# roymor1/OptimalStrategiesAgainstGenerativeAttacks

Measured on AMD Instinct MI355X. Metric: GIM episodes/sec (64x64x3, m=1 n=5 k=10), higher is better.
Workload: dtype f32

## Files before the change

### include/gim_hip.h

```cpp
#ifndef GIM_HIP_H
#define GIM_HIP_H

#include <stddef.h>
#include <stdint.h>

#ifdef __cplusplus
extern "C" {
#endif

#define GIM_OK 0
#define GIM_E_BADARG (-1)
#define GIM_E_LAUNCH (-2)

const char* gim_last_error(void);
int gim_version(void);

typedef struct {
    int32_t N, H, W, Cin, Cout, KH, ups;
    float pre_slope;
    int32_t pool, wfold, res_ups;
    int32_t tune_tile, tune_ksplit, tune_wgrad;
    int32_t out_zeroed;
    float post_slope;
    int32_t prec;
} gim_conv_shape;

int gim_conv2d_fold_weights(const float* w, float* f, int Cout, int Cin, int KH, void* stream);
typedef struct {
    const float* w;
    float* f;
    int32_t Cout, Cin, KH, reserved;
} gim_fold_job;
int gim_conv2d_fold_weights_batched(const gim_fold_job* jobs, const int32_t* tab, int n_blocks, void* stream);

int gim_conv2d_fwd(const float* x, const float* w, const float* bias, const float* sigma, const float* residual,
                   float* y, const gim_conv_shape* s, void* stream);

int gim_conv2d_dgrad(const float* dy, const float* w, const float* sigma, const float* mask_x, float* dx,
                     const gim_conv_shape* s, void* stream);

int gim_conv2d_dgrad_res(const float* dy, const float* w, const float* sigma, const float* mask_x, const float* res_half,
                         float res_scale, float* dx, const gim_conv_shape* s, void* stream);

int gim_conv2d_wgrad_slabs(const gim_conv_shape* s);
int gim_conv2d_wgrad(const float* dy, const float* x, float* slabs, float* bias_slabs, int n_slabs, const gim_conv_shape* s,
                     void* stream);

int gim_wgrad_finish(const float* slabs, const float* bias_slabs, int n_slabs, const float* w, const float* sigma,
                     const float* u, const float* v, float* dw, float* db, float* scratch, int Cout, int Cin, int KH,
                     int fold, float* acc_dw, float* acc_db, void* stream);

int gim_spectral_sigma(const float* w, float* u, float* v, float* sigma, float* u_out, float* v_out, float* scratch,
                       int Cout, int Cin, int KH, int training, void* stream);

typedef struct {
    const float* w;
    float* u;
    float* v;
    int64_t off_sigma, off_u, off_v, off_scratch;
    int32_t Cout, Cin, KH, reserved;
} gim_sn_job;
int gim_spectral_sigma_batched(const gim_sn_job* jobs, int n_jobs, const int32_t* tab_cols, int n_col_blocks,
                               const int32_t* tab_rows, int n_row_blocks, float* out_base, int training, void* stream);

int gim_conv2d_transpose_weights(const float* w, float* wt, int Cout, int Cin, int KF, void* stream);
int gim_conv2d_dgrad_t(const float* dy, const float* wt, const float* sigma, const float* mask_x, float* dx,
                       const gim_conv_shape* shape, void* stream);

int gim_conv2d_xfold_weights(const float* w, float* wx, int Cout, int Cin, int KH, int J, void* stream);
int gim_conv2d_dgrad_xfold(const float* dy, const float* wx, const float* sigma, const float* mask_x, float* dx,
                           const gim_conv_shape* shape, int J, void* stream);

int gim_pad_image(const float* x, float* xp, int N, int H, int W, int C, int pad, float slope, void* stream);
int gim_conv2d_pack_rows_weights(const float* w, float* wp, int Cout, int Cin, int KH, void* stream);
int gim_conv2d_fwd_rows(const float* xp, const float* wp, const float* bias, const float* sigma, const float* residual,
                        float* y, const gim_conv_shape* shape, void* stream);
int gim_conv2d_wgrad_rows_acc(const float* dy, const float* xp, float* acc, float* bias_acc, const gim_conv_shape* shape, void* stream);

int gim_conv2d_pack_subpixel_weights(const float* wf, float* wm, int Cout, int Cin, int KH, void* stream);
int gim_depth_to_space2(const float* y4, const float* bias, float* y, int N, int Hs, int Ws, int C, float post_slope, void* stream);

int gim_conv_launch_plan(const gim_conv_shape* shape, int kind, int32_t* out);

int gim_conv2d_wgrad_acc(const float* dy, const float* x, float* acc, float* bias_acc, const gim_conv_shape* shape, void* stream);

typedef struct {
    const float* src;
    const float* bias_src;
    const float* w;
    const float* sigma;
    const float* u;
    const float* v;
    float* tmp;
    float* partial;
    float* grad_w;
    float* grad_b;
    int32_t Cout, Cin, K, fold;
    int32_t n_chunks, exclusive;
} gim_wgrad_job;
int gim_wgrad_finish_batched(const gim_wgrad_job* jobs, int n_jobs, const int32_t* tab, int n_blocks, const int32_t* tab_sn,
                             int n_blocks_sn, void* stream);

int gim_colsum(const float* x, float* out, float* scratch, int64_t rows, int C, void* stream);

int gim_colsum_acc(const float* x, float* out, float* scratch, int64_t rows, int C, void* stream);
int gim_colsum2(const float* a, const float* b, float* out_a, float* out_b, int rows, int C, int accumulate, void* stream);

int gim_norm_fwd(const float* x, const float* scale, const float* shift, const float* residual, float* y, float* stats,
                 int N, int HW, int C, int mode, float eps, void* stream);
int gim_norm_fwd_act(const float* x, const float* scale, const float* shift, const float* residual, float* y, float* stats,
                     int N, int HW, int C, int mode, float eps, float post_slope, void* stream);
int gim_norm_bwd(const float* dy, const float* x, const float* scale, const float* stats, float* dx, float* dscale_nc,
                 float* dshift_nc, int N, int HW, int C, int mode, void* stream);

int gim_avgpool2_fwd(const float* x, float* y, int N, int H, int W, int C, void* stream);
int gim_avgpool2_fwd_act(const float* x, float* y, int N, int H, int W, int C, float in_slope, void* stream);
int gim_add_n(const float* a, const float* b, const float* c, const float* d, float* out, int64_t n, void* stream);
int gim_add_avgpool2_bwd(const float* g, const float* dy_pooled, float* out, int N, int H, int W, int C, void* stream);
int gim_avgpool2_bwd(const float* dy, float* dx, int N, int H, int W, int C, void* stream);
int gim_upsample2x_bwd(const float* dy_up, const float* mask_x, float slope, float* dx, int N, int H, int W, int C, void* stream);

int gim_maxpool_lrelu_fwd(const float* x, float* y, int32_t* idx, int N, int HW, int C, float slope, void* stream);
int gim_maxpool_lrelu_bwd(const float* dy, const float* y, const int32_t* idx, float* dx, int N, int HW, int C, float slope, void* stream);

int gim_attn_prob_fwd(const float* f, const float* g, float* P, int batch, int T, int K, void* stream);

int gim_bgemm(const float* A, const float* B, float* C, int batch, int M, int N, int K,
              int64_t sAb, int64_t sAi, int64_t sAk, int64_t sBb, int64_t sBk, int64_t sBj, void* stream);

typedef struct {
    const float* A;
    const float* B;
    float* C;
    const float* bias;
    int32_t M, N, K, ldc;
    int64_t sAi, sAk, sBk, sBj;
    int32_t flags, reserved;
} gim_gemm_job;
int gim_bgemm_grouped(const gim_gemm_job* jobs, const int32_t* tiles, int n_tiles, void* stream);
int gim_colsum_grouped(const gim_gemm_job* jobs, const int32_t* tiles, int n_tiles, void* stream);

int gim_softmax_dim1_fwd(const float* s, float* p, int B, int R, int Ccols, void* stream);
int gim_softmax_dim1_bwd(const float* dp, const float* p, float* ds, int B, int R, int Ccols, void* stream);

// ... 89 lines not shown
```

### optimalstrategiesagainstgenerativeattacks_amd/_lib.py

```python
import ctypes
import os
from ctypes import POINTER, c_float, c_int, c_int32, c_int64, c_void_p

_HERE = os.path.dirname(os.path.abspath(__file__))
LIB_PATH = os.environ.get("GIM_LIB_PATH") or os.path.join(_HERE, "csrc", "libgim_hip.so")


class GimConvShape(ctypes.Structure):
    _fields_ = [("N", c_int32), ("H", c_int32), ("W", c_int32), ("Cin", c_int32), ("Cout", c_int32),
                ("KH", c_int32), ("ups", c_int32), ("pre_slope", c_float),
                ("pool", c_int32), ("wfold", c_int32), ("res_ups", c_int32),
                ("tune_tile", c_int32), ("tune_ksplit", c_int32), ("tune_wgrad", c_int32),
                ("out_zeroed", c_int32), ("post_slope", c_float), ("prec", c_int32)]


class GimInferConv(ctypes.Structure):
    _fields_ = [("N", c_int32), ("H", c_int32), ("W", c_int32), ("Cin", c_int32), ("Cout", c_int32),
                ("KH", c_int32), ("stride", c_int32)]


P = c_void_p
SP = POINTER(GimConvShape)


class GimFoldJob(ctypes.Structure):
    _fields_ = [("w", P), ("f", P), ("Cout", c_int32), ("Cin", c_int32), ("KH", c_int32), ("reserved", c_int32)]


class GimSnJob(ctypes.Structure):
    _fields_ = [("w", P), ("u", P), ("v", P), ("off_sigma", c_int64), ("off_u", c_int64), ("off_v", c_int64), ("off_scratch", c_int64),
                ("Cout", c_int32), ("Cin", c_int32), ("KH", c_int32), ("reserved", c_int32)]


class GimWgradJob(ctypes.Structure):
    _fields_ = [("src", P), ("bias_src", P), ("w", P), ("sigma", P), ("u", P), ("v", P), ("tmp", P), ("partial", P),
                ("grad_w", P), ("grad_b", P), ("Cout", c_int32), ("Cin", c_int32), ("K", c_int32), ("fold", c_int32),
                ("n_chunks", c_int32), ("exclusive", c_int32)]


class GimGemmJob(ctypes.Structure):
    _fields_ = [("A", P), ("B", P), ("C", P), ("bias", P), ("M", c_int32), ("N", c_int32), ("K", c_int32), ("ldc", c_int32),
                ("sAi", c_int64), ("sAk", c_int64), ("sBk", c_int64), ("sBj", c_int64), ("flags", c_int32), ("reserved", c_int32)]


SIGNATURES = {
    "gim_conv2d_fwd": [P, P, P, P, P, P, SP, P],
    "gim_conv2d_dgrad": [P, P, P, P, P, SP, P],
    "gim_conv2d_dgrad_res": [P, P, P, P, P, c_float, P, SP, P],
    "gim_conv2d_wgrad_slabs": [SP],
    "gim_conv2d_wgrad": [P, P, P, P, c_int, SP, P],
    "gim_wgrad_finish": [P, P, c_int, P, P, P, P, P, P, P, c_int, c_int, c_int, c_int, P, P, P],
    "gim_conv2d_fold_weights": [P, P, c_int, c_int, c_int, P],
    "gim_conv2d_fold_weights_batched": [P, P, c_int, P],
    "gim_spectral_sigma": [P, P, P, P, P, P, P, c_int, c_int, c_int, c_int, P],
    "gim_spectral_sigma_batched": [P, c_int, P, c_int, P, c_int, P, c_int, P],
    "gim_colsum": [P, P, P, c_int64, c_int, P],
    "gim_norm_fwd": [P, P, P, P, P, P, c_int, c_int, c_int, c_int, c_float, P],
    "gim_norm_fwd_act": [P, P, P, P, P, P, c_int, c_int, c_int, c_int, c_float, c_float, P],
    "gim_norm_bwd": [P, P, P, P, P, P, P, c_int, c_int, c_int, c_int, P],
    "gim_avgpool2_fwd": [P, P, c_int, c_int, c_int, c_int, P],
    "gim_avgpool2_fwd_act": [P, P, c_int, c_int, c_int, c_int, c_float, P],
    "gim_add_n": [P, P, P, P, P, c_int64, P],
    "gim_add_avgpool2_bwd": [P, P, P, c_int, c_int, c_int, c_int, P],
    "gim_avgpool2_bwd": [P, P, c_int, c_int, c_int, c_int, P],
    "gim_upsample2x_bwd": [P, P, c_float, P, c_int, c_int, c_int, c_int, P],
    "gim_maxpool_lrelu_fwd": [P, P, P, c_int, c_int, c_int, c_float, P],
    "gim_maxpool_lrelu_bwd": [P, P, P, P, c_int, c_int, c_int, c_float, P],
    "gim_bgemm": [P, P, P, c_int, c_int, c_int, c_int, c_int64, c_int64, c_int64, c_int64, c_int64, c_int64, P],
    "gim_attn_prob_fwd": [P, P, P, c_int, c_int, c_int, P],
    "gim_softmax_dim1_fwd": [P, P, c_int, c_int, c_int, P],
    "gim_softmax_dim1_bwd": [P, P, P, c_int, c_int, c_int, P],
    "gim_bgemm_grouped": [P, P, c_int, P],
    "gim_colsum_grouped": [P, P, c_int, P],
    "gim_scale_add_fwd": [P, P, P, P, c_int64, P],
    "gim_scale_add_fwd_act": [P, P, P, P, c_int64, c_float, P],
    "gim_scale_add_bwd": [P, P, P, P, P, P, c_int64, P],
    "gim_tanh_fwd": [P, P, c_int64, P],
    "gim_tanh_bwd": [P, P, P, c_int64, P],
    "gim_nchw_to_nhwc": [P, P, c_int, c_int, c_int, P],
    "gim_nhwc_to_nchw": [P, P, c_int, c_int, c_int, P],
    "gim_set_stats_fwd": [P, P, P, c_int, c_int, c_int, c_int64, c_int64, P],
    "gim_set_stats_bwd": [P, P, P, P, c_int, c_int, c_int, c_int64, c_int64, P],
    "gim_bce_logits_fwd": [P, P, c_float, c_int, P],
    "gim_bce_logits_bwd": [P, P, P, c_float, c_int, P],
    "gim_sum_dim1": [P, P, c_int, c_int, c_int, c_float, P],
    "gim_repeat_dim1": [P, P, c_int, c_int, c_int, c_float, P],
    "gim_noise_combine": [P, P, P, c_int, c_int, c_int, c_int, P],
    "gim_concat2": [P, P, P, c_int64, c_int, c_int, c_int, c_int, P],
    "gim_slice_channels": [P, P, c_int64, c_int, c_int, P],
    "gim_conv2d_wgrad_acc": [P, P, P, P, SP, P],
    "gim_wgrad_finish_batched": [P, c_int, P, c_int, P, c_int, P],
    "gim_colsum_acc": [P, P, P, c_int64, c_int, P],
    "gim_colsum2": [P, P, P, P, c_int, c_int, c_int, P],
    "gim_conv_launch_plan": [SP, c_int, P],
    "gim_conv2d_transpose_weights": [P, P, c_int, c_int, c_int, P],
    "gim_conv2d_dgrad_t": [P, P, P, P, P, SP, P],
    "gim_conv2d_xfold_weights": [P, P, c_int, c_int, c_int, c_int, P],
    "gim_conv2d_dgrad_xfold": [P, P, P, P, P, SP, c_int, P],
    "gim_episode_gather": [P, P, P, P, c_int, c_int, c_int, c_int, P],
    "gim_resize_bilinear_u8": [P, c_int64, c_int, c_int, c_int, c_int, P, c_int, c_int, P, P, c_int, P, P, c_int, P],
    "gim_maxpool_gather": [P, P, P, P, c_int, c_int, c_int, c_float, P],
    "gim_softmax_dim1_bwd_dp": [P, P, P, P, c_int, c_int, c_int, P],
    "gim_set_stats_bwd_bwd": [P, P, P, P, P, P, c_int, c_int, c_int, c_int64, c_int64, P],
    "gim_lrelu_mask_mul": [P, P, c_float, P, c_int64, P],
    "gim_sqsum_rows_fwd": [P, P, c_int, c_int64, P],
    "gim_sqsum_rows_bwd": [P, P, P, c_int, c_int64, P],
    "gim_img_att_mix_fwd": [P, P, P, P, P, P, P, P, c_int64, c_int, P],
    "gim_img_att_mix_bwd": [P, P, P, P, P, P, P, P, P, P, P, P, P, P, c_int64, c_int, P],
    "gim_adam_step": [P, P, P, P, c_int64, P, P, c_int, c_float, c_float, c_float, c_float, P, P],
    "gim_adam_step_scaled": [P, P, P, P, c_int64, P, P, c_int, c_float, c_float, c_float, c_float, P, P, P],
    "gim_spin": [c_int, P],
    "gim_pad_image": [P, P, c_int, c_int, c_int, c_int, c_int, c_float, P],
    "gim_conv2d_pack_rows_weights": [P, P, c_int, c_int, c_int, P],
    "gim_conv2d_pack_subpixel_weights": [P, P, c_int, c_int, c_int, P],
    "gim_depth_to_space2": [P, P, P, c_int, c_int, c_int, c_int, c_float, P],
    "gim_conv2d_fwd_rows": [P, P, P, P, P, P, SP, P],
    "gim_conv2d_wgrad_rows_acc": [P, P, P, P, SP, P],
    "gim_conv2d_infer": [P, P, P, P, P, POINTER(GimInferConv), P],
    "gim_maxpool2_act": [P, P, c_int, c_int, c_int, c_int, c_int, P],
    "gim_channel_affine": [P, P, P, P, c_int64, c_int, P],
    "gim_se_tail": [P, P, P, P, P, P, P, c_int, c_int, c_int, c_int, c_int, P],
    "gim_pair_score": [P, P, P, c_int, c_int, P],
    "gim_l2norm_rows": [P, P, c_int, c_int, P],
    "gim_absdiff": [P, P, P, c_int64, P],
    "gim_bn_slabs": [c_int64],
    "gim_bn_partials_floats": [c_int64, c_int],
    "gim_bn_stats": [P, P, P, P, P, P, P, c_int64, c_int, c_float, c_float, P],
    "gim_bn_relu_maxpool2_fwd": [P, P, P, P, P, P, c_int, c_int, c_int, c_int, P],
    "gim_bn_pool_bwd_reduce": [P, P, P, P, P, P, P, P, P, P, P, c_int, c_int, c_int, c_int, P],
    "gim_bn_pool_bwd_dx": [P, P, P, P, P, P, P, P, P, c_int, c_int, c_int, c_int, P],
    "gim_absdiff_bwd": [P, P, P, P, P, c_int64, P],
    "gim_logit_accuracy": [P, c_int, c_int, P, P],
    "gim_version": [],
}

_lib = None


# ... 24 lines not shown
```

### optimalstrategiesagainstgenerativeattacks_amd/csrc/spectral.hip

```cpp
#include "common.h"

#define SN_R 8

__global__ __launch_bounds__(256) void sn_colpart_kernel(const float* __restrict__ w, const float* __restrict__ u,
                                                         float* __restrict__ part, int Cout, int K, int rows_per) {
    const int p = blockIdx.x * 256 + threadIdx.x;
    const int r = blockIdx.y;
    const int c0 = r * rows_per, c1 = min(Cout, c0 + rows_per);
    if (p >= K) return;
    float acc = 0.f;
    for (int co = c0; co < c1; ++co) acc += w[(long long)co * K + p] * u[co];
    part[(long long)r * K + p] = acc;
}

__global__ __launch_bounds__(256) void sn_vnorm_kernel(const float* __restrict__ part, int R, float* __restrict__ v,
                                                       float* __restrict__ v_phys, float* __restrict__ v_out, int K, int Cin,
                                                       int T, int training) {
    __shared__ float red[4];
    if (training) {
        float ss = 0.f;
        for (int p = threadIdx.x; p < K; p += 256) {
            float a = 0.f;
            for (int r = 0; r < R; ++r) a += part[(long long)r * K + p];
            v_phys[p] = a;
// ... 137 lines not shown
        const int kh = (int)(rr % K);
        const int co = (int)(rr / K);
        float g = 0.f;
#pragma unroll
        for (int dh = 0; dh < 2; ++dh)
#pragma unroll
            for (int dwd = 0; dwd < 2; ++dwd) {
                const int a = kh + dh, b = kw + dwd;
                if (fold == 1) g += src[(((long long)co * KF + a) * KF + b) * Cin + ci];
                else g += src[(((long long)ci * KF + (K - a)) * KF + (K - b)) * Cout + co];
            }
        if (fold == 1) g *= 0.25f;
        dw[i] = g;
        if (w) dot += g * w[i];
    }
    if (partial) {
        dot = block_sum_256(dot, red);
        if (threadIdx.x == 0) partial[blockIdx.x] = dot;
    }
}

__global__ __launch_bounds__(256) void wgrad_sn_apply_kernel(const float* __restrict__ g, float* __restrict__ dw, int accumulate,
                                                             const float* __restrict__ partial, int n_part,
                                                             const float* __restrict__ sigma, const float* __restrict__ u,
                                                             const float* __restrict__ v, long long n, int Cin, int T) {
    __shared__ float red[4];
    float d = 0.f;
    for (int i = threadIdx.x; i < n_part; i += 256) d += partial[i];
    d = block_sum_256(d, red);
    const float s = sigma[0];
    const float inv = 1.0f / s;
    const float coef = d * inv * inv;
    const int K = Cin * T;
    for (long long i = (long long)blockIdx.x * 256 + threadIdx.x; i < n; i += (long long)gridDim.x * 256) {
        const int co = (int)(i / K);
        const int p = (int)(i - (long long)co * K);
        const int tap = p / Cin, ci = p - tap * Cin;
        const float val = g[i] * inv - coef * u[co] * v[ci * T + tap];
        dw[i] = accumulate ? dw[i] + val : val;
    }
}

extern "C" int gim_wgrad_finish(const float* slabs, const float* bias_slabs, int n_slabs, const float* w, const float* sigma,
                                const float* u, const float* v, float* dw, float* db, float* scratch, int Cout, int Cin, int KH,
                                int fold, float* acc_dw, float* acc_db, void* stream) {
    GIM_CHECK_ARG(slabs && dw && n_slabs > 0, "wgrad_finish: bad args");
    GIM_CHECK_ARG((!db && !acc_db) || bias_slabs, "wgrad_finish: db needs bias_slabs");
    GIM_CHECK_ARG(!sigma || (w && u && v && scratch), "wgrad_finish: spectral form needs w, u, v, scratch");
    GIM_CHECK_ARG(fold >= 0 && fold <= 2 && (!fold || scratch), "wgrad_finish: bad fold / missing scratch");
    hipStream_t st = (hipStream_t)stream;
    const int T = KH * KH;
    const long long n = (long long)Cout * Cin * T;
    int blocks = (int)((n + 1023) / 1024);
    if (blocks > WF_BLOCKS) blocks = WF_BLOCKS;
    if (blocks < 1) blocks = 1;
    int sblocks = (int)((n + 63) / 64);
    if (sblocks > WF_BLOCKS) sblocks = WF_BLOCKS;
    float* bias_out = acc_db ? acc_db : db;
    const int bias_acc = acc_db ? 1 : 0;
    const bool direct = !sigma && !fold && acc_dw;
    if (fold == 0) {
        hipLaunchKernelGGL(wgrad_sum_kernel, dim3(sblocks), dim3(256), 0, st, slabs, n_slabs, n, sigma ? w : nullptr,
                           direct ? acc_dw : dw, sigma ? scratch : nullptr, bias_slabs, bias_out, Cout, direct ? 1 : 0, bias_acc);
        blocks = sblocks;
    } else {
        const long long nf = (long long)Cout * Cin * (KH + 1) * (KH + 1);
        float* fsum = scratch + WF_BLOCKS;
        int fb = (int)((nf + 63) / 64);
        if (fb > WF_BLOCKS) fb = WF_BLOCKS;
        hipLaunchKernelGGL(wgrad_sum_kernel, dim3(fb), dim3(256), 0, st, slabs, n_slabs, nf, (const float*)nullptr, fsum,
                           (float*)nullptr, bias_slabs, bias_out, Cout, 0, bias_acc);
        hipLaunchKernelGGL(wgrad_unfold_kernel, dim3(blocks), dim3(256), 0, st, fsum, sigma ? w : nullptr, dw,
                           sigma ? scratch : nullptr, Cout, Cin, KH, fold);
    }
    if (sigma) {
        hipLaunchKernelGGL(wgrad_sn_apply_kernel, dim3(blocks), dim3(256), 0, st, dw, acc_dw ? acc_dw : dw, acc_dw ? 1 : 0, scratch,
                           blocks, sigma, u, v, n, Cin, T);
    } else if (acc_dw && !direct) {
        GIM_CHECK_ARG(false, "wgrad_finish: acc_dw without sigma is only supported for fold == 0");
    }
    return gim_check_launch("gim_wgrad_finish");
}

__global__ __launch_bounds__(256) void snb_colpart_kernel(const gim_sn_job* __restrict__ jobs, const int4* __restrict__ tab,
                                                          float* __restrict__ out_base) {
    const int4 e = tab[blockIdx.x];
    const gim_sn_job jb = jobs[e.x];
    const int K = jb.Cin * jb.KH * jb.KH;
    const int p = e.y * 256 + threadIdx.x;
    if (p >= K) return;
    const int c0 = e.z * e.w, c1 = min(jb.Cout, c0 + e.w);
    float acc = 0.f;
    for (int co = c0; co < c1; ++co) acc += jb.w[(long long)co * K + p] * jb.u[co];
    (out_base + jb.off_scratch)[(long long)e.z * K + p] = acc;
}

__global__ __launch_bounds__(1024) void snb_vnorm_kernel(const gim_sn_job* __restrict__ jobs, float* __restrict__ out_base, int training) {
    __shared__ float red[16];
    const gim_sn_job jb = jobs[blockIdx.x];
    const int T = jb.KH * jb.KH, K = jb.Cin * T;
    const int R = min(SN_R, (jb.Cout + 63) / 64);
    float* part = out_base + jb.off_scratch;
    float* v_phys = part + (long long)SN_R * K;
    float* v_out = out_base + jb.off_v;
    if (training) {
        float ss = 0.f;
        for (int p = threadIdx.x; p < K; p += 1024) {
            float a = 0.f;
            for (int r = 0; r < R; ++r) a += part[(long long)r * K + p];
            v_phys[p] = a;
            ss += a * a;
        }
        ss = wave_sum(ss);
        if ((threadIdx.x & 63) == 0) red[threadIdx.x >> 6] = ss;
        __syncthreads();
        float tot = 0.f;
#pragma unroll
        for (int i = 0; i < 16; ++i) tot += red[i];
        const float inv = 1.0f / fmaxf(sqrtf(tot), 1e-12f);
        for (int p = threadIdx.x; p < K; p += 1024) {
            const float val = v_phys[p] * inv;
            const int tap = p / jb.Cin, ci = p - tap * jb.Cin;
            const int q = ci * T + tap;
            v_phys[p] = val;
            jb.v[q] = val;
            v_out[q] = val;
        }
    } else {
        for (int q = threadIdx.x; q < K; q += 1024) {
            const int ci = q / T, tap = q - ci * T;
            const float val = jb.v[q];
            v_phys[tap * jb.Cin + ci] = val;
            v_out[q] = val;
        }
    }
}

__global__ __launch_bounds__(256) void snb_rowdot_kernel(const gim_sn_job* __restrict__ jobs, const int2* __restrict__ tab,
                                                         float* __restrict__ out_base) {
    const int2 e = tab[blockIdx.x];
    const gim_sn_job jb = jobs[e.x];
    const int K = jb.Cin * jb.KH * jb.KH;
    const int co = e.y * 4 + (threadIdx.x >> 6);
    const int lane = threadIdx.x & 63;
    if (co >= jb.Cout) return;
    const float* v_phys = out_base + jb.off_scratch + (long long)SN_R * K;
    float* tvec = out_base + jb.off_scratch + (long long)(SN_R + 1) * K;
    const float* row = jb.w + (long long)co * K;
    float acc = 0.f;
    for (int p = lane; p < K; p += 64) acc += row[p] * v_phys[p];
    acc = wave_sum(acc);
    if (lane == 0) tvec[co] = acc;
}

__global__ __launch_bounds__(256) void snb_final_kernel(const gim_sn_job* __restrict__ jobs, float* __restrict__ out_base, int training) {
    __shared__ float red[4];
    const gim_sn_job jb = jobs[blockIdx.x];
    const int K = jb.Cin * jb.KH * jb.KH;
    const float* tvec = out_base + jb.off_scratch + (long long)(SN_R + 1) * K;
    float* u_out = out_base + jb.off_u;
    float inv = 0.f;
    if (training) {
        float ss = 0.f;
        for (int c = threadIdx.x; c < jb.Cout; c += 256) ss += tvec[c] * tvec[c];
        inv = 1.0f / fmaxf(sqrtf(block_sum_256(ss, red)), 1e-12f);
    }
    float dot = 0.f;
    for (int c = threadIdx.x; c < jb.Cout; c += 256) {
        float uv;
        if (training) {
            uv = tvec[c] * inv;
            jb.u[c] = uv;
        } else {
            uv = jb.u[c];
        }
        u_out[c] = uv;
        dot += uv * tvec[c];
    }
    dot = block_sum_256(dot, red);
    if (threadIdx.x == 0) (out_base + jb.off_sigma)[0] = dot;
}

extern "C" int gim_spectral_sigma_batched(const gim_sn_job* jobs, int n_jobs, const int32_t* tab_cols, int n_col_blocks,
                                          const int32_t* tab_rows, int n_row_blocks, float* out_base, int training, void* stream) {
    GIM_CHECK_ARG(jobs && n_jobs > 0 && tab_cols && tab_rows && out_base && n_col_blocks > 0 && n_row_blocks > 0,
                  "spectral_sigma_batched: bad args");
    hipStream_t st = (hipStream_t)stream;
    if (training)
        hipLaunchKernelGGL(snb_colpart_kernel, dim3(n_col_blocks), dim3(256), 0, st, jobs, reinterpret_cast<const int4*>(tab_cols), out_base);
    hipLaunchKernelGGL(snb_vnorm_kernel, dim3(n_jobs), dim3(1024), 0, st, jobs, out_base, training);
    hipLaunchKernelGGL(snb_rowdot_kernel, dim3(n_row_blocks), dim3(256), 0, st, jobs, reinterpret_cast<const int2*>(tab_rows), out_base);
    hipLaunchKernelGGL(snb_final_kernel, dim3(n_jobs), dim3(256), 0, st, jobs, out_base, training);
    return gim_check_launch("gim_spectral_sigma_batched");
}

#define WGQ_CHUNK 4096

__device__ __forceinline__ float wgq_load(const gim_wgrad_job& jb, unsigned i) {
    if (jb.fold == 0) return jb.src[i];
    const unsigned K = jb.K, KF = K + 1, Cin = jb.Cin, Cout = jb.Cout;
    const unsigned r1 = i / Cin, ci = i - r1 * Cin;
    const unsigned r2 = r1 / K, kw = r1 - r2 * K;
    if (jb.fold == 3)
        return jb.src[r2 * ((K * Cin + 15u) & ~15u) + kw * Cin + ci];
    const unsigned co = r2 / K, kh = r2 - co * K;
    float g = 0.f;
#pragma unroll
    for (unsigned dh = 0; dh < 2; ++dh)
#pragma unroll
        for (unsigned dwd = 0; dwd < 2; ++dwd) {
            const unsigned a = kh + dh, b = kw + dwd;
            if (jb.fold == 1) g += jb.src[((co * KF + a) * KF + b) * Cin + ci];
            else g += jb.src[((ci * KF + (K - a)) * KF + (K - b)) * Cout + co];
        }
    return jb.fold == 1 ? 0.25f * g : g;
}

__device__ __forceinline__ bool wgq_aligned16(const void* a, const void* b, const void* c) {
    return (((uintptr_t)a | (uintptr_t)b | (uintptr_t)c) & 15) == 0;
}

__global__ __launch_bounds__(256) void wgq_reduce_kernel(const gim_wgrad_job* __restrict__ jobs, const int2* __restrict__ tab) {
    __shared__ float red[4];
    const int2 e = tab[blockIdx.x];
    const gim_wgrad_job jb = jobs[e.x];
    const unsigned n = (unsigned)jb.Cout * jb.K * jb.K * jb.Cin;
    const unsigned i0 = (unsigned)e.y * WGQ_CHUNK;
    const unsigned cnt = min((unsigned)WGQ_CHUNK, n - i0);
    const bool sn = jb.sigma != nullptr;
    float dot = 0.f;
    if (sn && jb.fold == 2 && (jb.Cout & 63) == 0 && (jb.Cin & 63) == 0) {
        __shared__ float tile[64][65];
        const unsigned K = jb.K, KF = K + 1, T = K * K, Cin = jb.Cin, Cout = jb.Cout, tiles_ci = Cin >> 6;
        const unsigned tap = (unsigned)e.y % T, r = (unsigned)e.y / T;
        const unsigned ci0 = (r % tiles_ci) << 6, co0 = (r / tiles_ci) << 6;
        const unsigned kh = tap / K, kw = tap - kh * K;
        const unsigned lane = threadIdx.x & 63, wv = threadIdx.x >> 6;
#pragma unroll 4
        for (unsigned j = 0; j < 16; ++j) {
            const unsigned ci = ci0 + wv + 4 * j;
            const float* base = jb.src + (((size_t)ci * KF + (K - kh)) * KF + (K - kw)) * Cout + co0 + lane;
            tile[wv + 4 * j][lane] = (base[0] + base[-(long)Cout]) + (base[-(long)(KF * Cout)] + base[-(long)((KF + 1) * Cout)]);
        }
        __syncthreads();
#pragma unroll 4
        for (unsigned j = 0; j < 16; ++j) {
            const unsigned co = co0 + wv + 4 * j;
            const float g = tile[lane][wv + 4 * j];
            const unsigned i = ((co * K + kh) * K + kw) * Cin + ci0 + lane;
            jb.tmp[i] = g;
            dot += g * jb.w[i];
        }
    } else if (sn && jb.fold == 0 && (n & 3) == 0 && wgq_aligned16(jb.src, jb.w, jb.w)) {
        for (unsigned t = threadIdx.x * 4; t < cnt; t += 1024) {
            const float4 g = *reinterpret_cast<const float4*>(jb.src + i0 + t);
            const float4 w = *reinterpret_cast<const float4*>(jb.w + i0 + t);
            dot += g.x * w.x + g.y * w.y + g.z * w.z + g.w * w.w;
        }
    } else if (!sn && jb.fold == 0 && jb.exclusive && (n & 3) == 0 && wgq_aligned16(jb.src, jb.grad_w, jb.grad_w)) {
        for (unsigned t = threadIdx.x * 4; t < cnt; t += 1024) {
            const float4 g = *reinterpret_cast<const float4*>(jb.src + i0 + t);
            float4* dst = reinterpret_cast<float4*>(jb.grad_w + i0 + t);
            float4 o = *dst;
            o.x += g.x; o.y += g.y; o.z += g.z; o.w += g.w;
            *dst = o;
        }
    } else {
#pragma unroll 4
        for (unsigned t = threadIdx.x; t < cnt; t += 256) {
            const unsigned i = i0 + t;
            const float g = wgq_load(jb, i);
            if (sn) {
                if (jb.fold) jb.tmp[i] = g;
                dot += g * jb.w[i];
            } else {
                atomicAdd(&jb.grad_w[i], g);
// ... 73 lines not shown
```

### optimalstrategiesagainstgenerativeattacks_amd/model_blocks.py

```python
import collections
import math

import torch
import torch.nn as nn

from . import _lib
from . import ops

LRELU = 0.2


def _kaiming_uniform_like_torch(weight, bias, fan_in):
    nn.init.kaiming_uniform_(weight, a=math.sqrt(5))
    if bias is not None:
        bound = 1.0 / math.sqrt(fan_in) if fan_in > 0 else 0.0
        nn.init.uniform_(bias, -bound, bound)


class GimLinear(nn.Module):

    def __init__(self, in_features, out_features):
        super().__init__()
        self.in_features, self.out_features = in_features, out_features
        self.weight = nn.Parameter(torch.empty(out_features, in_features))
        self.bias = nn.Parameter(torch.empty(out_features))
        _kaiming_uniform_like_torch(self.weight, self.bias, in_features)

    def forward(self, x, pre_slope=1.0):
        return ops.linear(x, self.weight, self.bias, pre_slope)


class FusedLeakyReLU(nn.Module):

    def forward(self, x):
        raise RuntimeError("FusedLeakyReLU is fused into the next GimLinear")


class MLP(nn.Module):

    def __init__(self, layer_dims):
        super().__init__()
        assert len(layer_dims) >= 2
        layers = []
        inp_dim = layer_dims[0]
        for out_dim in layer_dims[1:-1]:
            layers.append(GimLinear(inp_dim, out_dim))
            layers.append(FusedLeakyReLU())
            inp_dim = out_dim
        layers.append(GimLinear(inp_dim, layer_dims[-1]))
        self.model = nn.Sequential(*layers)

    def forward(self, x):
        slope = 1.0
        for layer in self.model:
            if isinstance(layer, FusedLeakyReLU):
                slope = LRELU
            else:
                x = layer(x, pre_slope=slope)
                slope = 1.0
        return x


class SNConv2d(nn.Module):

    def __init__(self, in_channels, out_channels, kernel_size, padding=0):
        super().__init__()
        assert padding == (kernel_size - 1) // 2, "only 'same' stride-1 convolutions are on the GIM hot path"
        self.in_channels, self.out_channels, self.kernel_size = in_channels, out_channels, kernel_size
        w = torch.empty(out_channels, in_channels, kernel_size, kernel_size)
        b = torch.empty(out_channels)
        _kaiming_uniform_like_torch(w, b, in_channels * kernel_size * kernel_size)
        u = nn.functional.normalize(w.new_empty(out_channels).normal_(0, 1), dim=0, eps=1e-12)
        v = nn.functional.normalize(w.new_empty(in_channels * kernel_size * kernel_size).normal_(0, 1), dim=0, eps=1e-12)
        self.bias = nn.Parameter(b)
        self.weight_orig = nn.Parameter(w.contiguous(memory_format=torch.channels_last))
        self.register_buffer("weight_u", u)
        self.register_buffer("weight_v", v)

        self._sn_queue = collections.deque()
        self._wants_fold = False
        self._fold_slot = (kernel_size + 1, "fold")

    def fold_is_stale(self):
        return ops._WT_CACHE.is_stale(self.weight_orig, self._fold_slot)

    def folded(self):
        self._wants_fold = True
        return ops._WT_CACHE.get(self.weight_orig, self._fold_slot, lambda: ops._folded(
            ops.weight_phys(self.weight_orig), self.out_channels, self.in_channels, self.kernel_size))

    def forward(self, x, res=None, ups=0, pre_slope=1.0, pool=False, res_ups=False, post_slope=1.0, x_act=False, fork_pool_slope=None):
        guard = None
        if self._sn_queue:
            sigma, u_s, v_s, guard = self._sn_queue.popleft()
        else:
            sigma, u_s, v_s = ops.spectral_sigma(self.weight_orig, self.weight_u, self.weight_v, self.training)
        if fork_pool_slope is not None:
            assert res is None and not ups and not pool and not res_ups
            return ops.conv2d_forkpool(x, self.weight_orig, self.bias, sigma, u_s, v_s, pre_slope, guard, post_slope, x_act, fork_pool_slope)
        wf = self.folded() if (pool or (ups and self.kernel_size > 1)) else None
        if post_slope != 1.0:
            return ops.conv2d_post_act(x, self.weight_orig, self.bias, res, sigma, u_s, v_s, ups, pre_slope, pool, res_ups, wf, guard, post_slope, x_act)
        return ops.conv2d(x, self.weight_orig, self.bias, res, sigma, u_s, v_s, ups, pre_slope, pool, res_ups, wf, guard, x_act)

    def extra_repr(self):
        return "%d, %d, kernel_size=%d (spectral norm)" % (self.in_channels, self.out_channels, self.kernel_size)


class SNPlan:

    def __init__(self, convs):
        self.convs = [c for c in convs if isinstance(c, SNConv2d)]
        self._gen = 0
        self._bufs = {}
        self._tables = ops._TableCache("SNPlan", 1)
        self._fold_tables = ops._TableCache("SNPlan folds", None, skip_in_capture=True)

    def stale(self, gen):
        return self._gen - gen > 2

    def _build(self):
        jobs = (_lib.GimSnJob * len(self.convs))()
        cols, rows, views = [], [], []
        off = 0

        def take(n):
            nonlocal off
            o = off
            off += (n + 3) // 4 * 4
            return o
        for j, c in enumerate(self.convs):
            Cout, Cin, KH = c.out_channels, c.in_channels, c.kernel_size
            K = Cin * KH * KH
            if not c.weight_orig.permute(0, 2, 3, 1).is_contiguous():
                raise RuntimeError("SNPlan: weight_orig must be stored channels-last")
            o_s, o_u, o_v, o_scr = take(1), take(Cout), take(K), take(10 * K + Cout)
            jobs[j] = (c.weight_orig.data_ptr(), c.weight_u.data_ptr(), c.weight_v.data_ptr(), o_s, o_u, o_v, o_scr, Cout, Cin, KH, 0)
            R = min(8, (Cout + 63) // 64)
            rows_per = (Cout + R - 1) // R
            for xb in range((K + 255) // 256):
                for r in range(R):
                    cols.append((j, xb, r, rows_per))
            for rb in range((Cout + 3) // 4):
                rows.append((j, rb))
            views.append((o_s, o_u, Cout, o_v, K))
        return ops._DeviceTable(jobs, cols, rows, extra=(len(jobs), len(cols), len(rows), off, views))

    @torch.no_grad()
    def run(self, rounds, training):
        if not self.convs:
            return
        w0 = self.convs[0].weight_orig
        if not (w0.is_cuda and w0.dtype == torch.float32):
            raise RuntimeError("weights must be CUDA float32 (got %s on %s): the GIM engine has no CPU path" % (w0.dtype, w0.device))
        tab = self._tables.get(tuple(t.data_ptr() for c in self.convs for t in (c.weight_orig, c.weight_u, c.weight_v)), self._build)
        (d_jobs, d_cols, d_rows), (n_jobs, n_cols, n_rows, total, views) = tab.ptrs, tab.extra
        raw = ops._stream()
        tab.use_on_current_stream(raw)
        for c in self.convs:
            c._sn_queue.clear()
        gen = self._gen
        self._gen += 1
        for r in range(rounds):
            out = self._bufs.get((gen & 1, r))
            if out is None or out.numel() != total or out.device != w0.device:
                out = self._bufs[(gen & 1, r)] = torch.empty(total, device=w0.device, dtype=torch.float32)
            _lib.check(_lib.load().gim_spectral_sigma_batched(d_jobs, n_jobs, d_cols, n_cols, d_rows, n_rows, out.data_ptr(), 1 if training else 0, raw),
                       "spectral_sigma_batched")
            for c, (o_s, o_u, Cout, o_v, K) in zip(self.convs, views):
                c._sn_queue.append((out[o_s:o_s + 1], out[o_u:o_u + Cout], out[o_v:o_v + K], (self, gen)))
        self._fold_stale(raw)

    def _fold_stale(self, raw):
        todo = [c for c in self.convs if c._wants_fold and c.fold_is_stale()]
        if len(todo) < 2:
            return

        def build():
            jobs = (_lib.GimFoldJob * len(todo))()
            bufs, chunks = [], []
            for j, c in enumerate(todo):
                KF = c.kernel_size + 1
                n = c.out_channels * KF * KF * c.in_channels
                if n >= 1 << 31:
                    raise RuntimeError("folded weights of more than 2^31 elements (gim_conv2d_fold_weights_batched indexes with 32 bits)")
                bufs.append(torch.empty(n, device=c.weight_orig.device, dtype=torch.float32))
                jobs[j] = (c.weight_orig.data_ptr(), bufs[j].data_ptr(), c.out_channels, c.in_channels, c.kernel_size, 0)
                chunks += [(j, ch) for ch in range((n + 65535) // 65536)]
            return ops._DeviceTable(jobs, chunks, extra=(len(chunks), bufs))
        tab = self._fold_tables.get(tuple(c.weight_orig.data_ptr() for c in todo), build)
        if tab is None:
            return
        tab.use_on_current_stream(raw)
        _lib.check(_lib.load().gim_conv2d_fold_weights_batched(tab.ptrs[0], tab.ptrs[1], tab.extra[0], raw), "fold_weights_batched")
        for c, f in zip(todo, tab.extra[1]):
            ops._WT_CACHE.install(c.weight_orig, c._fold_slot, f)


def sn_convs(*modules):
    return [m for mod in modules for m in mod.modules() if isinstance(m, SNConv2d)]


class GimInstanceNorm2d(nn.Module):

    def __init__(self, num_features, eps=1e-5):
        super().__init__()
        self.num_features, self.eps = num_features, eps
        self.weight = nn.Parameter(torch.ones(num_features))
        self.bias = nn.Parameter(torch.zeros(num_features))

    def forward(self, x, post_slope=1.0):
        return ops.instance_norm(x, self.weight, self.bias, self.eps, post_slope)


def custom_std(x):
    D = x.shape[-1]
    return ops.mean_std_cat(x)[:, D:]


class ResBlockDown(nn.Module):

    def __init__(self, in_channel, out_channel, conv_size=3, padding_size=1):
        super().__init__()
        self.conv_l1 = SNConv2d(in_channel, out_channel, 1)
        self.conv_r1 = SNConv2d(in_channel, out_channel, conv_size, padding=padding_size)
        self.conv_r2 = SNConv2d(out_channel, out_channel, conv_size, padding=padding_size)

    def forward(self, x):
        return self.forward_act(x)[0]

    def forward_act(self, x, x_act=False, post_slope=1.0):
        out, act, pooled = self.conv_r1(x, pre_slope=LRELU, post_slope=LRELU, x_act=x_act, fork_pool_slope=LRELU if x_act else 1.0)
        left = self.conv_l1(pooled)
        if post_slope != 1.0 and ops.act_storage():
            return self.conv_r2(out, res=left, pre_slope=LRELU, pool=True, x_act=act, post_slope=post_slope)
        return self.conv_r2(out, res=left, pre_slope=LRELU, pool=True, x_act=act), False


class SelfAttention(nn.Module):

    def __init__(self, in_channel):
        super().__init__()
        self.conv_f = SNConv2d(in_channel, in_channel // 8, 1)
        self.conv_g = SNConv2d(in_channel, in_channel // 8, 1)
        self.conv_h = SNConv2d(in_channel, in_channel, 1)
        self.gamma = nn.Parameter(torch.zeros(1))

    def forward(self, x, post_slope=1.0):
        N, H, W, C = x.shape
        xf, xg, xh, xr = ops.fork(x, 4)
        f = self.conv_f(xf).view(N, H * W, -1)
# ... 107 lines not shown
```

Baseline: 434.7.

## Restructure batched spectral-norm power iteration and launch all rounds in one call

Replaces the four-kernel spectral sigma pipeline (column partials, v-normalise, row dots, final) with three kernels. W^T u is computed per 64-wide strip with float4 loads and shared-memory u chunks, and the per-strip sum of squares is kept so normalisation of v is folded into the later kernels. The W v row-dot kernel processes four rows per wave, or 64 rows per block for short K. A new rounds entry point issues every power-iteration round from one host call. This aims to cut kernel launches, scratch memory traffic and ctypes overhead, at the cost of more complex indexing and a different floating-point summation order.

```diff
diff --git a/include/gim_hip.h b/include/gim_hip.h
--- a/include/gim_hip.h
+++ b/include/gim_hip.h
@@ -60,6 +60,9 @@
     int64_t off_sigma, off_u, off_v, off_scratch;
     int32_t Cout, Cin, KH, reserved;
 } gim_sn_job;
+int gim_spectral_sigma_rounds(const gim_sn_job* jobs, int n_jobs, const int32_t* tab_cols, int n_col_blocks,
+                              const int32_t* tab_rows, int n_row_blocks, float* const* out_bases, int rounds, int training,
+                              void* stream);
 int gim_spectral_sigma_batched(const gim_sn_job* jobs, int n_jobs, const int32_t* tab_cols, int n_col_blocks,
                                const int32_t* tab_rows, int n_row_blocks, float* out_base, int training, void* stream);
 
diff --git a/optimalstrategiesagainstgenerativeattacks_amd/_lib.py b/optimalstrategiesagainstgenerativeattacks_amd/_lib.py
--- a/optimalstrategiesagainstgenerativeattacks_amd/_lib.py
+++ b/optimalstrategiesagainstgenerativeattacks_amd/_lib.py
@@ -54,6 +54,7 @@
     "gim_conv2d_fold_weights_batched": [P, P, c_int, P],
     "gim_spectral_sigma": [P, P, P, P, P, P, P, c_int, c_int, c_int, c_int, P],
     "gim_spectral_sigma_batched": [P, c_int, P, c_int, P, c_int, P, c_int, P],
+    "gim_spectral_sigma_rounds": [P, c_int, P, c_int, P, c_int, P, c_int, c_int, P],
     "gim_colsum": [P, P, P, c_int64, c_int, P],
     "gim_norm_fwd": [P, P, P, P, P, P, c_int, c_int, c_int, c_int, c_float, P],
     "gim_norm_fwd_act": [P, P, P, P, P, P, c_int, c_int, c_int, c_int, c_float, c_float, P],
diff --git a/optimalstrategiesagainstgenerativeattacks_amd/csrc/spectral.hip b/optimalstrategiesagainstgenerativeattacks_amd/csrc/spectral.hip
--- a/optimalstrategiesagainstgenerativeattacks_amd/csrc/spectral.hip
+++ b/optimalstrategiesagainstgenerativeattacks_amd/csrc/spectral.hip
@@ -243,94 +243,222 @@
     return gim_check_launch("gim_wgrad_finish");
 }
 
-__global__ __launch_bounds__(256) void snb_colpart_kernel(const gim_sn_job* __restrict__ jobs, const int4* __restrict__ tab,
-                                                          float* __restrict__ out_base) {
+#define SNB_STRIP 64
+#define SNB_ROWS 4
+#define SNB_UCHUNK 1024
+
+struct snb_scratch {
+    float* a;
+    float* ssq;
+    float* t;
+};
+
+__device__ __forceinline__ int snb_strips(int K) { return (K + SNB_STRIP - 1) / SNB_STRIP; }
+
+__device__ __forceinline__ snb_scratch snb_scratch_of(const gim_sn_job& jb, float* out_base, int K) {
+    snb_scratch sc;
+    sc.a = out_base + jb.off_scratch;
+    sc.ssq = sc.a + ((K + 3) & ~3);
+    sc.t = sc.ssq + ((snb_strips(K) + 3) & ~3);
+    return sc;
+}
+
+__device__ __forceinline__ bool snb_vec(const gim_sn_job& jb, const float* a, int K) {
+    return (K & 3) == 0 && (((uintptr_t)jb.w | (uintptr_t)a) & 15) == 0;
+}
+
+__device__ __forceinline__ float snb_inv_norm(const snb_scratch& sc, int K) {
+    const int ns = snb_strips(K);
+    float ss = 0.f;
+    for (int i = threadIdx.x & 63; i < ns; i += 64) ss += sc.ssq[i];
+    return 1.0f / fmaxf(sqrtf(wave_sum(ss)), 1e-12f);
+}
+
+__device__ __forceinline__ float dot4(const float4 a, const float4 b) { return (a.x * b.x + a.y * b.y) + (a.z * b.z + a.w * b.w); }
+
+__global__ __launch_bounds__(256) void snb_wtu_kernel(const gim_sn_job* __restrict__ jobs, const int2* __restrict__ tab,
+                                                      float* __restrict__ out_base) {
+    __shared__ float su[SNB_UCHUNK];
+    __shared__ float red[16][SNB_STRIP];
+    const int2 e = tab[blockIdx.x];
+    const gim_sn_job jb = jobs[e.x];
+    const int K = jb.Cin * jb.KH * jb.KH, Cout = jb.Cout;
+    const snb_scratch sc = snb_scratch_of(jb, out_base, K);
+    const bool vec = snb_vec(jb, sc.a, K);
+    const int tid = threadIdx.x;
+    const int p0 = e.y * SNB_STRIP;
+    const int cl = vec ? (tid & 15) : (tid & 63), rg = vec ? (tid >> 4) : (tid >> 6);
+    const int p = p0 + (vec ? cl * 4 : cl);
+    const bool on = p < K;
+    float4 acc = make_float4(0.f, 0.f, 0.f, 0.f);
+    for (int c0 = 0; c0 < Cout; c0 += SNB_UCHUNK) {
+        const int n = min(SNB_UCHUNK, Cout - c0);
+        __syncthreads();
+        for (int i = tid; i < n; i += 256) su[i] = jb.u[c0 + i];
+        __syncthreads();
+        if (!on) continue;
+        const float* wp = jb.w + (size_t)c0 * K + p;
+        int r = rg;
+        if (vec) {
+            for (; r + 16 * 7 < n; r += 16 * 8) {
+                float4 x[8];
+#pragma unroll
+                for (int i = 0; i < 8; ++i) x[i] = *reinterpret_cast<const float4*>(wp + (size_t)(r + 16 * i) * K);
+#pragma unroll
+                for (int i = 0; i < 8; ++i) {
+                    const float uu = su[r + 16 * i];
+                    acc.x += x[i].x * uu; acc.y += x[i].y * uu; acc.z += x[i].z * uu; acc.w += x[i].w * uu;
+                }
+            }
+            for (; r < n; r += 16) {
+                const float4 x = *reinterpret_cast<const float4*>(wp + (size_t)r * K);
+                const float uu = su[r];
+                acc.x += x.x * uu; acc.y += x.y * uu; acc.z += x.z * uu; acc.w += x.w * uu;
+            }
+        } else {
+            for (; r + 4 * 7 < n; r += 4 * 8) {
+                float x[8];
+#pragma unroll
+                for (int i = 0; i < 8; ++i) x[i] = wp[(size_t)(r + 4 * i) * K];
+#pragma unroll
+                for (int i = 0; i < 8; ++i) acc.x += x[i] * su[r + 4 * i];
+            }
+            for (; r < n; r += 4) acc.x += wp[(size_t)r * K] * su[r];
+        }
+    }
+    if (vec) {
+        red[rg][cl * 4 + 0] = acc.x; red[rg][cl * 4 + 1] = acc.y; red[rg][cl * 4 + 2] = acc.z; red[rg][cl * 4 + 3] = acc.w;
+    } else {
+        red[rg][cl] = acc.x;
+    }
+    __syncthreads();
+    if (tid < SNB_STRIP) {
+        const int groups = vec ? 16 : 4;
+        float a = 0.f;
+        for (int g = 0; g < groups; ++g) a += red[g][tid];
+        if (p0 + tid < K) sc.a[p0 + tid] = a;
+        else a = 0.f;
+        const float ss = wave_sum(a * a);
+        if (tid == 0) sc.ssq[e.y] = ss;
+    }
+}
+
+__global__ __launch_bounds__(SNB_STRIP) void snb_vload_kernel(const gim_sn_job* __restrict__ jobs, const int2* __restrict__ tab,
+                                                              float* __restrict__ out_base) {
+    const int2 e = tab[blockIdx.x];
+    const gim_sn_job jb = jobs[e.x];
+    const int T = jb.KH * jb.KH, K = jb.Cin * T;
+    const int p = e.y * SNB_STRIP + threadIdx.x;
+    if (p >= K) return;
+    const int tap = p / jb.Cin, ci = p - tap * jb.Cin;
+    const int q = ci * T + tap;
+    const float val = jb.v[q];
+    snb_scratch_of(jb, out_base, K).a[p] = val;
+    (out_base + jb.off_v)[q] = val;
+}
+
+__global__ __launch_bounds__(256) void snb_wv_kernel(const gim_sn_job* __restrict__ jobs, const int4* __restrict__ tab,
+                                                     float* __restrict__ out_base, int training) {
+    __shared__ float red[4][SNB_ROWS];
     const int4 e = tab[blockIdx.x];
     const gim_sn_job jb = jobs[e.x];
-    const int K = jb.Cin * jb.KH * jb.KH;
-    const int p = e.y * 256 + threadIdx.x;
-    if (p >= K) return;
-    const int c0 = e.z * e.w, c1 = min(jb.Cout, c0 + e.w);
-    float acc = 0.f;
-    for (int co = c0; co < c1; ++co) acc += jb.w[(long long)co * K + p] * jb.u[co];
-    (out_base + jb.off_scratch)[(long long)e.z * K + p] = acc;
-}
-
-__global__ __launch_bounds__(1024) void snb_vnorm_kernel(const gim_sn_job* __restrict__ jobs, float* __restrict__ out_base, int training) {
-    __shared__ float red[16];
-    const gim_sn_job jb = jobs[blockIdx.x];
-    const int T = jb.KH * jb.KH, K = jb.Cin * T;
-    const int R = min(SN_R, (jb.Cout + 63) / 64);
-    float* part = out_base + jb.off_scratch;
-    float* v_phys = part + (long long)SN_R * K;
-    float* v_out = out_base + jb.off_v;
-    if (training) {
-        float ss = 0.f;
-        for (int p = threadIdx.x; p < K; p += 1024) {
-            float a = 0.f;
-            for (int r = 0; r < R; ++r) a += part[(long long)r * K + p];
-            v_phys[p] = a;
-            ss += a * a;
-        }
-        ss = wave_sum(ss);
-        if ((threadIdx.x & 63) == 0) red[threadIdx.x >> 6] = ss;
-        __syncthreads();
-        float tot = 0.f;
-#pragma unroll
-        for (int i = 0; i < 16; ++i) tot += red[i];
-        const float inv = 1.0f / fmaxf(sqrtf(tot), 1e-12f);
-        for (int p = threadIdx.x; p < K; p += 1024) {
-            const float val = v_phys[p] * inv;
+    const int T = jb.KH * jb.KH, K = jb.Cin * T, Cout = jb.Cout;
+    const snb_scratch sc = snb_scratch_of(jb, out_base, K);
+    const bool vec = snb_vec(jb, sc.a, K);
+    const int tid = threadIdx.x, lane = tid & 63, wv = tid >> 6;
+    const int r_end = min(Cout, e.y + e.z);
+    const float4* a4 = reinterpret_cast<const float4*>(sc.a);
+    const int K4 = K >> 2;
+    if (vec && e.w) {
+        const int l = tid & 15, g = tid >> 4;
+        for (int r0 = e.y + g * SNB_ROWS; r0 < r_end; r0 += 16 * SNB_ROWS) {
+            const float4* w4[SNB_ROWS];
+            float acc[SNB_ROWS];
+#pragma unroll
+            for (int j = 0; j < SNB_ROWS; ++j) {
+                w4[j] = reinterpret_cast<const float4*>(jb.w + (size_t)min(r0 + j, Cout - 1) * K);
+                acc[j] = 0.f;
+            }
+            for (int k = l; k < K4; k += 16) {
+                const float4 av = a4[k];
+#pragma unroll
+                for (int j = 0; j < SNB_ROWS; ++j) acc[j] += dot4(w4[j][k], av);
+            }
+#pragma unroll
+            for (int j = 0; j < SNB_ROWS; ++j) {
+                float s = acc[j];
+#pragma unroll
+                for (int o = 8; o > 0; o >>= 1) s += __shfl_xor(s, o, 64);
+                if (l == 0 && r0 + j < r_end) sc.t[r0 + j] = s;
+            }
+        }
+    } else {
+        for (int r0 = e.y; r0 < r_end; r0 += SNB_ROWS) {
+            const float* w[SNB_ROWS];
+            float acc[SNB_ROWS];
+#pragma unroll
+            for (int j = 0; j < SNB_ROWS; ++j) {
+                w[j] = jb.w + (size_t)min(r0 + j, Cout - 1) * K;
+                acc[j] = 0.f;
+            }
+            if (vec) {
+#pragma unroll 2
+                for (int k = tid; k < K4; k += 256) {
+                    const float4 av = a4[k];
+#pragma unroll
+                    for (int j = 0; j < SNB_ROWS; ++j) acc[j] += dot4(reinterpret_cast<const float4*>(w[j])[k], av);
+                }
+            } else {
+#pragma unroll 2
+                for (int k = tid; k < K; k += 256) {
+                    const float av = sc.a[k];
+#pragma unroll
+                    for (int j = 0; j < SNB_ROWS; ++j) acc[j] += w[j][k] * av;
+                }
+            }
+#pragma unroll
+            for (int j = 0; j < SNB_ROWS; ++j) acc[j] = wave_sum(acc[j]);
+            __syncthreads();
+            if (lane == 0) {
+#pragma unroll
+                for (int j = 0; j < SNB_ROWS; ++j) red[wv][j] = acc[j];
+            }
+            __syncthreads();
+            if (tid < SNB_ROWS && r0 + tid < r_end) sc.t[r0 + tid] = (red[0][tid] + red[1][tid]) + (red[2][tid] + red[3][tid]);
+        }
+    }
+    if (training && e.y == 0) {
+        const float inv = snb_inv_norm(sc, K);
+        float* v_out = out_base + jb.off_v;
+        for (int p = tid; p < K; p += 256) {
             const int tap = p / jb.Cin, ci = p - tap * jb.Cin;
             const int q = ci * T + tap;
-            v_phys[p] = val;
+            const float val = sc.a[p] * inv;
             jb.v[q] = val;
             v_out[q] = val;
         }
-    } else {
-        for (int q = threadIdx.x; q < K; q += 1024) {
-            const int ci = q / T, tap = q - ci * T;
-            const float val = jb.v[q];
-            v_phys[tap * jb.Cin + ci] = val;
-            v_out[q] = val;
-        }
-    }
-}
-
-__global__ __launch_bounds__(256) void snb_rowdot_kernel(const gim_sn_job* __restrict__ jobs, const int2* __restrict__ tab,
-                                                         float* __restrict__ out_base) {
-    const int2 e = tab[blockIdx.x];
-    const gim_sn_job jb = jobs[e.x];
-    const int K = jb.Cin * jb.KH * jb.KH;
-    const int co = e.y * 4 + (threadIdx.x >> 6);
-    const int lane = threadIdx.x & 63;
-    if (co >= jb.Cout) return;
-    const float* v_phys = out_base + jb.off_scratch + (long long)SN_R * K;
-    float* tvec = out_base + jb.off_scratch + (long long)(SN_R + 1) * K;
-    const float* row = jb.w + (long long)co * K;
-    float acc = 0.f;
-    for (int p = lane; p < K; p += 64) acc += row[p] * v_phys[p];
-    acc = wave_sum(acc);
-    if (lane == 0) tvec[co] = acc;
+    }
 }
 
 __global__ __launch_bounds__(256) void snb_final_kernel(const gim_sn_job* __restrict__ jobs, float* __restrict__ out_base, int training) {
     __shared__ float red[4];
     const gim_sn_job jb = jobs[blockIdx.x];
     const int K = jb.Cin * jb.KH * jb.KH;
-    const float* tvec = out_base + jb.off_scratch + (long long)(SN_R + 1) * K;
+    const snb_scratch sc = snb_scratch_of(jb, out_base, K);
+    const float* tvec = sc.t;
     float* u_out = out_base + jb.off_u;
-    float inv = 0.f;
+    float s = 1.f, scale = 0.f;
     if (training) {
+        s = snb_inv_norm(sc, K);
         float ss = 0.f;
         for (int c = threadIdx.x; c < jb.Cout; c += 256) ss += tvec[c] * tvec[c];
-        inv = 1.0f / fmaxf(sqrtf(block_sum_256(ss, red)), 1e-12f);
+        scale = s / fmaxf(sqrtf(block_sum_256(ss, red)) * s, 1e-12f);
     }
     float dot = 0.f;
     for (int c = threadIdx.x; c < jb.Cout; c += 256) {
         float uv;
         if (training) {
-            uv = tvec[c] * inv;
+            uv = tvec[c] * scale;
             jb.u[c] = uv;
         } else {
             uv = jb.u[c];
@@ -339,20 +467,31 @@
         dot += uv * tvec[c];
     }
     dot = block_sum_256(dot, red);
-    if (threadIdx.x == 0) (out_base + jb.off_sigma)[0] = dot;
+    if (threadIdx.x == 0) (out_base + jb.off_sigma)[0] = dot * s;
+}
+
+extern "C" int gim_spectral_sigma_rounds(const gim_sn_job* jobs, int n_jobs, const int32_t* tab_cols, int n_col_blocks,
+                                         const int32_t* tab_rows, int n_row_blocks, float* const* out_bases, int rounds,
+                                         int training, void* stream) {
+    GIM_CHECK_ARG(jobs && n_jobs > 0 && tab_cols && tab_rows && out_bases && n_col_blocks > 0 && n_row_blocks > 0 && rounds > 0,
+                  "spectral_sigma_rounds: bad args");
+    for (int r = 0; r < rounds; ++r) GIM_CHECK_ARG(out_bases[r], "spectral_sigma_rounds: null output base");
+    hipStream_t st = (hipStream_t)stream;
+    const int2* cols = reinterpret_cast<const int2*>(tab_cols);
+    const int4* rows = reinterpret_cast<const int4*>(tab_rows);
+    for (int r = 0; r < rounds; ++r) {
+        float* out = out_bases[r];
+        if (training) hipLaunchKernelGGL(snb_wtu_kernel, dim3(n_col_blocks), dim3(256), 0, st, jobs, cols, out);
+        else hipLaunchKernelGGL(snb_vload_kernel, dim3(n_col_blocks), dim3(SNB_STRIP), 0, st, jobs, cols, out);
+        hipLaunchKernelGGL(snb_wv_kernel, dim3(n_row_blocks), dim3(256), 0, st, jobs, rows, out, training);
+        hipLaunchKernelGGL(snb_final_kernel, dim3(n_jobs), dim3(256), 0, st, jobs, out, training);
+    }
+    return gim_check_launch("gim_spectral_sigma_rounds");
 }
 
 extern "C" int gim_spectral_sigma_batched(const gim_sn_job* jobs, int n_jobs, const int32_t* tab_cols, int n_col_blocks,
                                           const int32_t* tab_rows, int n_row_blocks, float* out_base, int training, void* stream) {
-    GIM_CHECK_ARG(jobs && n_jobs > 0 && tab_cols && tab_rows && out_base && n_col_blocks > 0 && n_row_blocks > 0,
-                  "spectral_sigma_batched: bad args");
-    hipStream_t st = (hipStream_t)stream;
-    if (training)
-        hipLaunchKernelGGL(snb_colpart_kernel, dim3(n_col_blocks), dim3(256), 0, st, jobs, reinterpret_cast<const int4*>(tab_cols), out_base);
-    hipLaunchKernelGGL(snb_vnorm_kernel, dim3(n_jobs), dim3(1024), 0, st, jobs, out_base, training);
-    hipLaunchKernelGGL(snb_rowdot_kernel, dim3(n_row_blocks), dim3(256), 0, st, jobs, reinterpret_cast<const int2*>(tab_rows), out_base);
-    hipLaunchKernelGGL(snb_final_kernel, dim3(n_jobs), dim3(256), 0, st, jobs, out_base, training);
-    return gim_check_launch("gim_spectral_sigma_batched");
+    return gim_spectral_sigma_rounds(jobs, n_jobs, tab_cols, n_col_blocks, tab_rows, n_row_blocks, &out_base, 1, training, stream);
 }
 
 #define WGQ_CHUNK 4096
diff --git a/optimalstrategiesagainstgenerativeattacks_amd/model_blocks.py b/optimalstrategiesagainstgenerativeattacks_amd/model_blocks.py
--- a/optimalstrategiesagainstgenerativeattacks_amd/model_blocks.py
+++ b/optimalstrategiesagainstgenerativeattacks_amd/model_blocks.py
@@ -1,4 +1,5 @@
 import collections
+import ctypes
 import math
 
 import torch
@@ -134,15 +135,13 @@
             K = Cin * KH * KH
             if not c.weight_orig.permute(0, 2, 3, 1).is_contiguous():
                 raise RuntimeError("SNPlan: weight_orig must be stored channels-last")
-            o_s, o_u, o_v, o_scr = take(1), take(Cout), take(K), take(10 * K + Cout)
+            strips = (K + 63) // 64
+            o_s, o_u, o_v, o_scr = take(1), take(Cout), take(K), take((K + 3) // 4 * 4 + (strips + 3) // 4 * 4 + Cout)
             jobs[j] = (c.weight_orig.data_ptr(), c.weight_u.data_ptr(), c.weight_v.data_ptr(), o_s, o_u, o_v, o_scr, Cout, Cin, KH, 0)
-            R = min(8, (Cout + 63) // 64)
-            rows_per = (Cout + R - 1) // R
-            for xb in range((K + 255) // 256):
-                for r in range(R):
-                    cols.append((j, xb, r, rows_per))
-            for rb in range((Cout + 3) // 4):
-                rows.append((j, rb))
+            cols += [(j, s) for s in range(strips)]
+            short = K <= 256 and K % 4 == 0
+            rows_per = 64 if short else 4
+            rows += [(j, r0, min(rows_per, Cout - r0), int(short)) for r0 in range(0, Cout, rows_per)]
             views.append((o_s, o_u, Cout, o_v, K))
         return ops._DeviceTable(jobs, cols, rows, extra=(len(jobs), len(cols), len(rows), off, views))
 
@@ -161,12 +160,17 @@
             c._sn_queue.clear()
         gen = self._gen
         self._gen += 1
+        outs = []
         for r in range(rounds):
             out = self._bufs.get((gen & 1, r))
             if out is None or out.numel() != total or out.device != w0.device:
                 out = self._bufs[(gen & 1, r)] = torch.empty(total, device=w0.device, dtype=torch.float32)
-            _lib.check(_lib.load().gim_spectral_sigma_batched(d_jobs, n_jobs, d_cols, n_cols, d_rows, n_rows, out.data_ptr(), 1 if training else 0, raw),
-                       "spectral_sigma_batched")
+            outs.append(out)
+        bases = (ctypes.c_void_p * len(outs))(*(o.data_ptr() for o in outs))
+        if outs:
+            _lib.check(_lib.load().gim_spectral_sigma_rounds(d_jobs, n_jobs, d_cols, n_cols, d_rows, n_rows, bases, len(outs), 1 if training else 0, raw),
+                       "spectral_sigma_rounds")
+        for out in outs:
             for c, (o_s, o_u, Cout, o_v, K) in zip(self.convs, views):
                 c._sn_queue.append((out[o_s:o_s + 1], out[o_u:o_u + Cout], out[o_v:o_v + K], (self, gen)))
         self._fold_stale(raw)
```

Result: no change. 435.9, median of 5 (+0.3%).
